# jby1993/SelfReconCode

Measured on AMD Instinct MI355X. Metric: train.py-equivalent iterations/sec (540x540, 2048 rays/frame x 3 frames per GPU; coarse stage at Adam lr 0.0001), higher is better.
Workload: dtype f32

## Files before the change

include/selfrecon_hip.h:

```cpp
#ifndef SELFRECON_HIP_H_
#define SELFRECON_HIP_H_
#include <stdint.h>

#ifdef __cplusplus
extern "C" {
#endif

#define SR_OK 0
#define SR_EINVAL (-1)
#define SR_ELAUNCH (-2)
#define SR_ENOSPC (-3)

int sr_abi_version(void);
const char* sr_build_arch(void);
const char* sr_build_digest(void);

int sr_minv3x3_fwd_f32(const float* ms, float* invs, uint8_t* checks, int64_t n, void* stream);
int sr_minv3x3_fwd_f64(const double* ms, double* invs, uint8_t* checks, int64_t n, void* stream);
int sr_minv3x3_bwd_f32(const float* grads, const float* invs, float* outs, int64_t n, void* stream);
int sr_minv3x3_bwd_f64(const double* grads, const double* invs, double* outs, int64_t n, void* stream);

typedef struct {
  int64_t size[5];
  int64_t stride[5];
// ... 19 lines not shown
                             void* grad_grad_output, void* stream);
int sr_gridsample3d_dbwd_f32(const float* gO_input , sr_tensor5 goi_d, const float* gO_grid, sr_tensor5 gog_d,
                             const float* input, sr_tensor5 in_d, const float* grid, sr_tensor5 grid_d,
                             const float* grad_output, sr_tensor5 gout_d,
                             float* grad_input , sr_tensor5 gin_d, float* grad_grid, float* grad_grad_output,
                             void* stream);
int sr_gridsample3d_dbwd_f64(const double* gO_input , sr_tensor5 goi_d, const double* gO_grid, sr_tensor5 gog_d,
                             const double* input, sr_tensor5 in_d, const double* grid, sr_tensor5 grid_d,
                             const double* grad_output, sr_tensor5 gout_d,
                             double* grad_input , sr_tensor5 gin_d, double* grad_grid, double* grad_grad_output,
                             void* stream);


#define SR_ACT_NONE 0
#define SR_ACT_SOFTPLUS100 1
#define SR_ACT_RELU 2
#define SR_EPI_FWD 0
#define SR_EPI_BWD 1
typedef struct {
  const float* A; int64_t lda;
  const float* B; int64_t ldb;
  float* C; int64_t ldc;
  int32_t M, N, K;
  const float* bias;
  int32_t group, act, mode;
  float out_scale;
  const float* aux; int64_t ldaux;
  int32_t naux_fwd;
  int32_t nact_bwd;
  float aux_scale;
} sr_gemm_args;
int sr_mlp_gemm_nt(const sr_gemm_args* host_args, void* stream);
int sr_mlp_gemm_nt_tile(int32_t M, int32_t ncols, int32_t* bm_out, int32_t* bn_out);

#define SR_CHAIN_MAX_LAYERS 10
typedef struct {
  int32_t nlayers;
  int32_t nprob[SR_CHAIN_MAX_LAYERS];
  sr_gemm_args g[SR_CHAIN_MAX_LAYERS][2];
  const int32_t* m_dev; int32_t m_mul;
  int32_t m_cap;
} sr_chain_args;
int sr_mlp_chain(const sr_chain_args* host_args, void* stream);

typedef struct {
  const float* Z; int64_t ldz;
  const float* A; int64_t lda;
  float* dW; int64_t lddw;
  float* partial;
  int32_t R, N, K, splits, accumulate;
  float* db; float* db_partial; int32_t group;
} sr_gemm_tn_args;
int64_t sr_mlp_gemm_tn_workspace_floats(int32_t R, int32_t N, int64_t lddw, int32_t* host_splits_out);
int sr_mlp_gemm_tn(const sr_gemm_tn_args* host_args, void* stream);
#define SR_TN_GROUP_MAX 12
typedef struct {
  int32_t n;
  sr_gemm_tn_args p[SR_TN_GROUP_MAX];
} sr_gemm_tn_group_args;
int sr_mlp_gemm_tn_group(const sr_gemm_tn_group_args* host_args, void* stream);

int sr_pe_embed(const float* x, int64_t P, int32_t L, const float* band_weights, const float* extra, int64_t ldextra,
                int32_t E, const int64_t* extra_index , int32_t group, float* out, int64_t ldo, void* stream);
int sr_pe_embed_bwd(const float* x, int64_t P, int32_t L, const float* band_weights, int32_t group, const float* gA0,
                    int64_t ldg, float* xbar, void* stream);

typedef struct {
  const float* p; const float* tp; int64_t P;
  const float* A; const float* trans; int32_t nframes;
  const int64_t* batch_inds; int64_t points_per_frame;
  const float* vol; int32_t D, H, W;
  float bmin[3], bmax[3];
  float* y;
  float* jac;
} sr_lbs_args;
int sr_lbs_fwd(const sr_lbs_args* host_args, void* stream);
int64_t sr_lbs_bwd_workspace_floats(int64_t P, int32_t nframes);
int sr_lbs_bwd(const sr_lbs_args* host_args, const float* ybar, float* pbar, float* Abar, float* transbar, float* partials, void* stream);
int sr_lbs_jac_bwd(const sr_lbs_args* host_args, const float* ybar, const float* Jbar, float* pbar, float* Abar, float* transbar, float* partials,
                   void* stream);

int sr_lbs_chain_fwd(const float* poses, int32_t B, const float* host_Js, const int32_t* host_parents, const float* host_init_pose,
                     float* G, float* A, void* stream);
int sr_lbs_chain_bwd(const float* poses, int32_t B, const float* host_Js, const int32_t* host_parents, const float* host_init_pose,
                     const float* Abar, const float* Gbar, float* posebar, void* stream);

typedef struct {
// ... 183 lines not shown
```

selfreconcode_amd/_lib.py:

```python
import ctypes
import os
import torch

from .build import LIB

_i64, _vp, _int = ctypes.c_int64, ctypes.c_void_p, ctypes.c_int


class SrTensor5(ctypes.Structure):
    _fields_ = [("size", _i64 * 5), ("stride", _i64 * 5)]


class SrGemmArgs(ctypes.Structure):
    _fields_ = [("A", _vp), ("lda", _i64), ("B", _vp), ("ldb", _i64), ("C", _vp), ("ldc", _i64),
                ("M", ctypes.c_int32), ("N", ctypes.c_int32), ("K", ctypes.c_int32), ("bias", _vp),
                ("group", ctypes.c_int32), ("act", ctypes.c_int32), ("mode", ctypes.c_int32), ("out_scale", ctypes.c_float),
                ("aux", _vp), ("ldaux", _i64), ("naux_fwd", ctypes.c_int32), ("nact_bwd", ctypes.c_int32),
                ("aux_scale", ctypes.c_float)]


class SrGemmTnArgs(ctypes.Structure):
    _fields_ = [("Z", _vp), ("ldz", _i64), ("A", _vp), ("lda", _i64), ("dW", _vp), ("lddw", _i64), ("partial", _vp),
                ("R", ctypes.c_int32), ("N", ctypes.c_int32), ("K", ctypes.c_int32), ("splits", ctypes.c_int32),
                ("accumulate", ctypes.c_int32), ("db", _vp), ("db_partial", _vp), ("group", ctypes.c_int32)]
# ... 98 lines not shown
_CODES = {-1: "SR_EINVAL (bad argument)", -2: "SR_ELAUNCH (kernel launch failed)", -3: "SR_ENOSPC (workspace too small)"}

if "SELFRECON_HIP_LIB" in os.environ:
    LIB = os.environ["SELFRECON_HIP_LIB"]
else:
    from .build import is_stale, build_lib
    if is_stale():
        try:
            build_lib(verbose=False)
        except RuntimeError as e:
            raise ImportError(str(e)) from e
if not os.path.isfile(LIB):
    raise ImportError(f"{LIB} not found: run `python -m selfreconcode_amd.build` (hipcc --offload-arch=gfx950). "
                      "There is no CPU fallback for the HIP hot path.")
_lib = ctypes.CDLL(LIB)

_T5 = SrTensor5
SIGNATURES = {
    "sr_minv3x3_fwd_f32": [_vp, _vp, _vp, _i64, _vp],
    "sr_minv3x3_fwd_f64": [_vp, _vp, _vp, _i64, _vp],
    "sr_minv3x3_bwd_f32": [_vp, _vp, _vp, _i64, _vp],
    "sr_minv3x3_bwd_f64": [_vp, _vp, _vp, _i64, _vp],
    "sr_gridsample3d_fwd_f16": [_vp, _T5, _vp, _T5, _vp, _T5, _vp],
    "sr_gridsample3d_bwd_f16": [_vp, _T5, _vp, _T5, _vp, _T5, _vp, _T5, _vp, _vp],
    "sr_gridsample3d_dbwd_f16": [_vp, _T5, _vp, _T5, _vp, _T5, _vp, _T5, _vp, _T5, _vp, _T5, _vp, _vp, _vp],
    "sr_gridsample3d_fwd_f32": [_vp, _T5, _vp, _T5, _vp, _T5, _vp],
    "sr_gridsample3d_fwd_f64": [_vp, _T5, _vp, _T5, _vp, _T5, _vp],
    "sr_gridsample3d_bwd_f32": [_vp, _T5, _vp, _T5, _vp, _T5, _vp, _T5, _vp, _vp],
    "sr_gridsample3d_bwd_f64": [_vp, _T5, _vp, _T5, _vp, _T5, _vp, _T5, _vp, _vp],
    "sr_gridsample3d_dbwd_f32": [_vp, _T5, _vp, _T5, _vp, _T5, _vp, _T5, _vp, _T5, _vp, _T5, _vp, _vp, _vp],
    "sr_gridsample3d_dbwd_f64": [_vp, _T5, _vp, _T5, _vp, _T5, _vp, _T5, _vp, _T5, _vp, _T5, _vp, _vp, _vp],
    "sr_mlp_gemm_nt": [_vp, _vp],
    "sr_mlp_gemm_nt_tile": [ctypes.c_int32, ctypes.c_int32, _vp, _vp],
    "sr_mlp_chain": [_vp, _vp],
    "sr_refine_init": [_vp, _vp],
    "sr_refine_embed": [_vp, ctypes.c_int32, _vp],
    "sr_refine_mid": [_vp, ctypes.c_int32, ctypes.c_int32, _vp],
    "sr_refine_finish": [_vp, ctypes.c_int32, _vp],
    "sr_mlp_gemm_tn_workspace_floats": [ctypes.c_int32, ctypes.c_int32, _i64, _vp],
    "sr_mlp_gemm_tn": [_vp, _vp],
    "sr_mlp_gemm_tn_group": [_vp, _vp],
    "sr_lbs_chain_fwd": [_vp, ctypes.c_int32, _vp, _vp, _vp, _vp, _vp, _vp],
    "sr_lbs_chain_bwd": [_vp, ctypes.c_int32, _vp, _vp, _vp, _vp, _vp, _vp, _vp],
    "sr_lbs_fwd": [_vp, _vp],
    "sr_lbs_bwd_workspace_floats": [_i64, ctypes.c_int32],
    "sr_lbs_bwd": [_vp, _vp, _vp, _vp, _vp, _vp, _vp],
    "sr_lbs_jac_bwd": [_vp, _vp, _vp, _vp, _vp, _vp, _vp, _vp],
    "sr_newton_update": [_vp, _vp],
    "sr_newton_prepare": [_vp, _vp],
    "sr_newton_apply": [_vp, _vp],
    "sr_mc_workspace_bytes": [ctypes.c_int32, ctypes.c_int32, ctypes.c_int32],
    "sr_mc_count": [_vp, ctypes.c_int32, ctypes.c_int32, ctypes.c_int32, ctypes.c_float, _vp, _vp, _vp],
    "sr_mc_emit": [_vp, ctypes.c_int32, ctypes.c_int32, ctypes.c_int32, ctypes.c_float, _vp] + [ctypes.c_float] * 6 + [_vp, _vp, _vp],
    "sr_rows_pad": [_vp, _i64, ctypes.c_int32, _vp, _i64, ctypes.c_int32, _i64, ctypes.c_int32, _vp, _i64, ctypes.c_int32, _vp],
    "sr_rows_frame_sum_workspace_floats": [_i64, ctypes.c_int32, ctypes.c_int32],
    "sr_rows_frame_sum": [_vp, _i64, _i64, ctypes.c_int32, _vp, ctypes.c_int32, _vp, _vp, _vp],
    "sr_adam_step": [_vp, _vp],
    "sr_stream_stamp": [_vp, _vp],
    "sr_stream_flag_set": [_vp, ctypes.c_uint32, _vp],
    "sr_stream_flag_wait": [_vp, ctypes.c_uint32, _vp, ctypes.c_int32, _vp],
    "sr_pack_weights": [_vp, _vp],
    "sr_unpack_grads": [_vp, _vp],
    "sr_svd3x3": [_vp, _i64, _vp, _vp, _vp, _vp],
    "sr_step_reduce_blocks": [_i64],
    "sr_step_param_blocks": [_i64],
    "sr_cam_project_ndc_fwd": [_vp, _i64, _vp, _vp, _vp, _vp],
    "sr_cam_project_ndc_bwd": [_vp, _i64, _vp, _vp, _vp, _vp, _vp, _vp, _vp],
    "sr_cam_view_rays_fwd": [_vp, _i64, _vp, _vp, _vp],
    "sr_cam_view_rays_bwd": [_vp, _i64, _vp, _vp, _vp, _vp, _vp],
    "sr_cardinal_rays_fwd": [_vp, _vp, _i64, _vp, _vp, _vp],
    "sr_cardinal_rays_bwd": [_vp, _vp, _i64, _vp, _vp, _vp, _vp],
    "sr_deformed_normals": [_vp, _vp, _i64, _vp, _vp],
    "sr_color_loss_fwd": [_vp, _vp, _vp, _vp, _vp, _vp],
# ... 172 lines not shown
```

selfreconcode_amd/csrc/mlp_gemm.hip:

```cpp
#include "sr_common.h"
#include <stdlib.h>
#include <type_traits>

typedef float f32x16 __attribute__((ext_vector_type(16)));
typedef float f32x4 __attribute__((ext_vector_type(4)));
typedef int i32x4 __attribute__((ext_vector_type(4)));

__device__ __forceinline__ __amdgpu_buffer_rsrc_t sr_make_rsrc(const void* base, int64_t bytes) {
  return __builtin_amdgcn_make_buffer_rsrc(const_cast<void*>(base), 0, (int)(bytes < 0xFFFFFFFFll ? bytes : 0xFFFFFFFFll), 0x00020000);
}
__device__ __forceinline__ f32x4 sr_buffer_load16(__amdgpu_buffer_rsrc_t rsrc, uint32_t lane_off, uint32_t scalar_off) {
  return __builtin_bit_cast(f32x4, __builtin_amdgcn_raw_buffer_load_b128(rsrc, (int)lane_off, (int)scalar_off, 0));
}

namespace {

constexpr int BK = 32;
constexpr int LDSP = BK + 4;

__device__ __forceinline__ float fast_exp(float x) { return __builtin_amdgcn_exp2f(x * 1.4426950408889634f); }
__device__ __forceinline__ float fast_log(float x) { return __builtin_amdgcn_logf(x) * 0.6931471805599453f; }
__device__ __forceinline__ float softplus100(float z) {
  const float t = z * 100.0f;
  const float e = fast_exp(fminf(t, 20.0f));
  const float l = e < 1e-3f ? e * (1.0f - e * (0.5f - e * 0.33333334f)) : fast_log(1.0f + e);
  return t > 20.0f ? z : l * 0.01f;
}
__device__ __forceinline__ float dsoftplus100(float z) {
  const float t = z * 100.0f;
  const float e = fast_exp(fminf(t, 20.0f));
  return t > 20.0f ? 1.0f : e * __builtin_amdgcn_rcpf(e + 1.0f);
}
__device__ __forceinline__ void softplus100_from_stored(float x, float& d, float& c2) {
  const float em = fast_exp(-x);
// ... 190 lines not shown
            if constexpr (ACT == SR_ACT_SOFTPLUS100) softplus100_from_stored(100.0f * (sv[s] * inv_as), d, c2);
            else if constexpr (ACT == SR_ACT_RELU) d = sv[s] > 0.f ? 1.f : 0.f;
            float cross = 0.f;
#pragma unroll
            for (int tI = 1; tI < G; ++tI) {
              cross += sv[s + tI] * v[s + tI];
              o[s + tI] = d * as * v[s + tI];
            }
            o[s] = d * as * v[s] + c2 * cross;
          }
        }
        float* sp = stage + (a * 32 + 8 * q + 4 * kh) * SP + b * 32 + li;
#pragma unroll
        for (int j = 0; j < 4; ++j) sp[j * SP] = o[j];
      }
    }
  }
  __syncthreads();
  constexpr int QPR = TN * 8, RPI = 64 / QPR;
  const int lane = kh * 32 + li;
  const int qc = lane % QPR, ro = lane / QPR;
  float* dst = g.C + (int64_t)(m0 + wm * TM * 32 + ro) * g.ldc + n0 + wn * TN * 32 + qc * 4;
#pragma unroll
  for (int i = 0; i < TM * 32 / RPI; ++i)
    *reinterpret_cast<f32x4*>(dst + (int64_t)i * RPI * g.ldc) = *reinterpret_cast<const f32x4*>(stage + (i * RPI + ro) * SP + qc * 4);
}

template <int WM, int WN, int TM, int TN, int G, int MODE>
__device__ __forceinline__ void epilogue_interior_act(const sr_gemm_args& g, f32x16 (&acc)[TM][TN], int m0, int n0, int wm, int wn, int li,
                                                      int kh, float* __restrict__ stage) {
  if (g.act == SR_ACT_SOFTPLUS100) epilogue_interior<WM, WN, TM, TN, G, MODE, SR_ACT_SOFTPLUS100>(g, acc, m0, n0, wm, wn, li, kh, stage);
  else if (g.act == SR_ACT_RELU) epilogue_interior<WM, WN, TM, TN, G, MODE, SR_ACT_RELU>(g, acc, m0, n0, wm, wn, li, kh, stage);
  else epilogue_interior<WM, WN, TM, TN, G, MODE, SR_ACT_NONE>(g, acc, m0, n0, wm, wn, li, kh, stage);
}

struct NoProbe { __device__ __forceinline__ void operator()(int) const {} };
template <int WM, int WN, int TM, int TN, bool KTAIL = true, class Probe = NoProbe>
__device__ __forceinline__ void gemm_nt_tile(const sr_gemm_args& g, int wg, float* __restrict__ smem, Probe probe = Probe()) {
  using C_ = Cfg<WM, WN, TM, TN>;
  auto As = [&](int buf) -> float* { return smem + buf * (C_::BM * LDSP); };
  auto Bs = [&](int buf) -> float* { return smem + 2 * C_::BM * LDSP + buf * (C_::BN * LDSP); };

  const int tiles_n = (g.N + g.naux_fwd + C_::BN - 1) / C_::BN;
  const int tiles_m = (g.M + C_::BM - 1) / C_::BM;
  const int nwg = tiles_m * tiles_n;
  {
    const int q = nwg / 8, r = nwg % 8, xcd = wg % 8, loc = wg / 8;
    wg = (xcd < r ? xcd * (q + 1) : r * (q + 1) + (xcd - r) * q) + loc;
  }
  const int tn = wg % tiles_n, tm = wg / tiles_n;
  const int m0 = tm * C_::BM, n0 = tn * C_::BN;

  const int lane = threadIdx.x & 63, wave = threadIdx.x >> 6;
  const int wm = wave / WN, wn = wave % WN;
  const int li = lane & 31, kh = lane >> 5;

  f32x16 acc[TM][TN];
#pragma unroll
  for (int a = 0; a < TM; ++a)
#pragma unroll
    for (int b = 0; b < TN; ++b)
#pragma unroll
      for (int r = 0; r < 16; ++r) acc[a][b][r] = 0.f;

  const TileLoader<C_::BM, C_::kALoads, C_::kThreads> la(g.A, g.lda, g.M, g.K, m0);
  const TileLoader<C_::BN, C_::kBLoads, C_::kThreads> lb(g.B, g.ldb, g.N, g.K, n0);
// ... 40 lines not shown
    mfma_kk(fa0[0], fb0[0]);
    mfma_kk(fa0[1], fb0[1]);
#pragma unroll
    for (int i = 0; i < kMem; ++i) {
      __builtin_amdgcn_sched_group_barrier(0x020, 1, 0);
      __builtin_amdgcn_sched_group_barrier(0x008, 1, 0);
    }
#pragma unroll
    for (int i = 0; i < kMem; ++i) {
      __builtin_amdgcn_sched_group_barrier(0x200, 1, 0);
      __builtin_amdgcn_sched_group_barrier(0x008, 1, 0);
    }
#pragma unroll
    for (int i = 0; i < 2 * (TM + TN); ++i) {
      __builtin_amdgcn_sched_group_barrier(0x100, 1, 0);
      __builtin_amdgcn_sched_group_barrier(0x008, 1, 0);
    }
    __builtin_amdgcn_sched_barrier(0);
    __syncthreads();
    read_frags(As(cur ^ 1), Bs(cur ^ 1), 0, fa0, fb0);
    __builtin_amdgcn_sched_barrier(0);
    mfma_kk(fa1[0], fb1[0]);
    mfma_kk(fa1[1], fb1[1]);
    __builtin_amdgcn_sched_barrier(0);
  };
  for (int t = 0; t < nk; t += 2) {
    step(t, ra0, rb0, ra1, rb1);
    if (t + 1 < nk) step(t + 1, ra1, rb1, ra0, rb0);
  }
  __syncthreads();
  probe(1);

  float* stage = smem + wave * (TM * 32 * (TN * 32 + 4));
  const bool interior = m0 + C_::BM <= g.M && n0 + C_::BN <= (g.mode == SR_EPI_FWD ? g.N : (g.nact_bwd < g.N ? g.nact_bwd : g.N));
  if (interior) {
    if (g.mode == SR_EPI_FWD) {
      switch (g.group) {
        case 1: epilogue_interior_act<WM, WN, TM, TN, 1, SR_EPI_FWD>(g, acc, m0, n0, wm, wn, li, kh, stage); break;
        case 2: epilogue_interior_act<WM, WN, TM, TN, 2, SR_EPI_FWD>(g, acc, m0, n0, wm, wn, li, kh, stage); break;
        default: epilogue_interior_act<WM, WN, TM, TN, 4, SR_EPI_FWD>(g, acc, m0, n0, wm, wn, li, kh, stage); break;
      }
    } else {
      switch (g.group) {
        case 1: epilogue_interior_act<WM, WN, TM, TN, 1, SR_EPI_BWD>(g, acc, m0, n0, wm, wn, li, kh, stage); break;
        case 2: epilogue_interior_act<WM, WN, TM, TN, 2, SR_EPI_BWD>(g, acc, m0, n0, wm, wn, li, kh, stage); break;
        default: epilogue_interior_act<WM, WN, TM, TN, 4, SR_EPI_BWD>(g, acc, m0, n0, wm, wn, li, kh, stage); break;
      }
    }
  } else {
    switch (g.group) {
      case 1: epilogue<WM, WN, TM, TN, 1>(g, acc, m0, n0, wm, wn, li, kh, stage); break;
      case 2: epilogue<WM, WN, TM, TN, 2>(g, acc, m0, n0, wm, wn, li, kh, stage); break;
      default: epilogue<WM, WN, TM, TN, 4>(g, acc, m0, n0, wm, wn, li, kh, stage); break;
    }
  }
  probe(2);
}

template <int WM, int WN, int TM, int TN, bool KTAIL>
__global__ __launch_bounds__(WM * WN * 64) __attribute__((amdgpu_waves_per_eu(2))) void gemm_nt_kernel(sr_gemm_args g) {
  extern __shared__ __attribute__((aligned(16))) float smem[];
  gemm_nt_tile<WM, WN, TM, TN, KTAIL>(g, blockIdx.x, smem);
}


using ChainCfg = Cfg<2, 2, 1, 1>;

constexpr int TBR = 32;
template <int ZW, int XW>
struct TnCfg {
  static constexpr int ZLD = ZW + 4, XLD = XW + 4;
  static constexpr int kZ = TBR * ZLD, kX = TBR * XLD;
  static constexpr int kLdsFloats = 2 * (kZ + kX);
  static constexpr int TLZ = TBR * (ZW / 4) / 256, TLX = TBR * (XW / 4) / 256;
  static constexpr int WN = XW / 64;
};

template <int ZW, int XW>
__device__ __forceinline__ void gemm_tn_body(const sr_gemm_tn_args& g, int rows_per_split, int bid, int nblocks, float* __restrict__ tn_smem) {
  using C = TnCfg<ZW, XW>;
  auto Zs = [&](int buf) -> float* { return tn_smem + buf * C::kZ; };
  auto Xs = [&](int buf) -> float* { return tn_smem + 2 * C::kZ + buf * C::kX; };
  const int tiles_k = (g.K + XW - 1) / XW;
  const int tiles_n = (g.N + ZW - 1) / ZW;
  int vb = bid;
  if ((nblocks & 7) == 0) vb = (bid & 7) * (nblocks >> 3) + (bid >> 3);
  const int tile = vb % (tiles_k * tiles_n), split = vb / (tiles_k * tiles_n);
  const int n0 = (tile / tiles_k) * ZW, k0 = (tile % tiles_k) * XW;
  const int r_begin = split * rows_per_split;
  const int r_end = min(g.R, r_begin + rows_per_split);
  const int lane = threadIdx.x & 63, wave = threadIdx.x >> 6;
  const int wm = wave / C::WN, wn = wave % C::WN, li = lane & 31, kh = lane >> 5;

  f32x16 acc[2][2];
#pragma unroll
  for (int a = 0; a < 2; ++a)
#pragma unroll
// ... 241 lines not shown
}

__global__ __launch_bounds__(256) void slab_reduce_group_kernel(TnGroup G) {
  int i = 0;
  while (i + 1 < G.n && (int)blockIdx.x >= G.first[i + 1]) ++i;
  const int bid = blockIdx.x - G.first[i];
  if (bid >= G.blocks[i]) return;
  const sr_gemm_tn_args& g = G.p[i];
  slab_reduce_body(g.partial, g.dW, g.N, g.K, g.lddw, g.R > 0 ? g.splits : 0, g.accumulate, g.db_partial, g.db, bid, G.blocks[i]);
}

}

static void nt_tile_choice(int M, int ncols, int* bm, int* bn) {
  auto cost = [&](int tm, int tn, double eff) {
    const int64_t wgs = sr_cdiv(M, tm) * sr_cdiv(ncols, tn);
    return (double)sr_cdiv(wgs, 256) * tm * tn / eff;
  };
  if (ncols <= 32) {
    const double c[3] = {cost(32, 32, 0.6), cost(64, 32, 0.8), cost(256, 32, 1.0)};
    *bn = 32;
    if (c[0] < c[1] && c[0] < c[2]) *bm = 32;
    else if (c[1] < c[2]) *bm = 64;
    else *bm = 256;
  } else {
    const double c[3] = {cost(64, 64, 0.92), cost(64, 128, 0.94), cost(128, 128, 1.0)};
    int pick = 1;
    for (int i = 1; i < 3; ++i) if (c[i] < c[pick - 1]) pick = i + 1;
    *bm = pick == 3 ? 128 : 64;
    *bn = pick == 1 ? 64 : 128;
  }
}

extern "C" {
int sr_mlp_gemm_nt(const sr_gemm_args* a, void* stream) {
  if (!a || a->M < 0 || a->N <= 0 || a->K <= 0) return SR_EINVAL;
  if (a->M == 0) return SR_OK;
  if (!a->A || !a->B || !a->C) return SR_EINVAL;
  if (a->group != 1 && a->group != 2 && a->group != 4) return SR_EINVAL;
  if ((a->lda & 3) || (a->ldb & 3) || (a->ldc & 3) || ((uintptr_t)a->A & 15) || ((uintptr_t)a->B & 15) || ((uintptr_t)a->C & 15)) return SR_EINVAL;
  if (a->mode != SR_EPI_FWD && a->mode != SR_EPI_BWD) return SR_EINVAL;
  if ((a->naux_fwd > 0 || a->mode == SR_EPI_BWD) && a->act != SR_ACT_NONE && !a->aux && a->mode == SR_EPI_BWD) return SR_EINVAL;
  if (a->mode == SR_EPI_FWD && a->naux_fwd > 0 && !a->aux) return SR_EINVAL;
  if (a->M == 0) return SR_OK;
  if (a->M % a->group) return SR_EINVAL;
  const int ncols = a->N + (a->mode == SR_EPI_FWD ? a->naux_fwd : 0);
  sr_gemm_args g = *a;
  if (g.mode != SR_EPI_FWD) g.naux_fwd = 0;
#define SR_NT_LAUNCH(WM, WN, TM, TN)                                                                                        \
  do {                                                                                                                      \
    using C_ = Cfg<WM, WN, TM, TN>;                                                                                         \
    const int nwg = (int)(sr_cdiv(g.M, C_::BM) * sr_cdiv(ncols, C_::BN));                                                   \
    if (g.K % BK)                                                                                                           \
      hipLaunchKernelGGL((gemm_nt_kernel<WM, WN, TM, TN, true>), dim3(nwg), dim3(C_::kThreads), C_::kLdsFloats * sizeof(float), \
                         (hipStream_t)stream, g);                                                                           \
    else                                                                                                                    \
      hipLaunchKernelGGL((gemm_nt_kernel<WM, WN, TM, TN, false>), dim3(nwg), dim3(C_::kThreads), C_::kLdsFloats * sizeof(float), \
                         (hipStream_t)stream, g);                                                                           \
  } while (0)
  int bm = 0, bn = 0;
  nt_tile_choice(g.M, ncols, &bm, &bn);
  switch (bm * 1024 + bn) {
    case 32 * 1024 + 32: SR_NT_LAUNCH(1, 1, 1, 1); break;
    case 64 * 1024 + 32: SR_NT_LAUNCH(2, 1, 1, 1); break;
    case 256 * 1024 + 32: SR_NT_LAUNCH(4, 1, 2, 1); break;
    case 64 * 1024 + 64: SR_NT_LAUNCH(2, 2, 1, 1); break;
    case 64 * 1024 + 128: SR_NT_LAUNCH(2, 2, 1, 2); break;
    default: SR_NT_LAUNCH(2, 2, 2, 2); break;
  }
#undef SR_NT_LAUNCH
  return sr_launch_status();
}

int sr_mlp_gemm_nt_tile(int32_t M, int32_t ncols, int32_t* bm, int32_t* bn) {
  if (M <= 0 || ncols <= 0 || !bm || !bn) return SR_EINVAL;
  nt_tile_choice(M, ncols, bm, bn);
  return SR_OK;
}

__global__ __launch_bounds__(ChainCfg::kThreads) __attribute__((amdgpu_waves_per_eu(2))) void mlp_layer_pair_kernel(sr_gemm_args g0, sr_gemm_args g1, int nprob,
                                                                                                                     const int32_t* __restrict__ m_dev, int m_mul) {
  extern __shared__ __attribute__((aligned(16))) float smem[];
  const int M = *m_dev * m_mul;
  if (M <= 0) return;
  const int rows = (M + ChainCfg::BM - 1) / ChainCfg::BM;
  const int t0 = rows * ((g0.N + (g0.mode == SR_EPI_FWD ? g0.naux_fwd : 0) + ChainCfg::BN - 1) / ChainCfg::BN);
  const int t1 = nprob > 1 ? rows * ((g1.N + (g1.mode == SR_EPI_FWD ? g1.naux_fwd : 0) + ChainCfg::BN - 1) / ChainCfg::BN) : 0;
  const int t = blockIdx.x;
  if (t >= t0 + t1) return;
  if (t < t0) { g0.M = M; if (g0.K % BK) gemm_nt_tile<2, 2, 1, 1, true>(g0, t, smem); else gemm_nt_tile<2, 2, 1, 1, false>(g0, t, smem); }
  else { g1.M = M; if (g1.K % BK) gemm_nt_tile<2, 2, 1, 1, true>(g1, t - t0, smem); else gemm_nt_tile<2, 2, 1, 1, false>(g1, t - t0, smem); }
}

int sr_mlp_chain(const sr_chain_args* a, void* stream) {
  if (!a || a->nlayers < 1 || a->nlayers > SR_CHAIN_MAX_LAYERS || !a->m_dev || a->m_mul < 1 || a->m_cap <= 0) return SR_EINVAL;
  for (int l = 0; l < a->nlayers; ++l) {
    if (a->nprob[l] < 1 || a->nprob[l] > 2) return SR_EINVAL;
    for (int p = 0; p < a->nprob[l]; ++p) {
      const sr_gemm_args& g = a->g[l][p];
      if (!g.A || !g.B || !g.C || g.N <= 0 || g.K <= 0 || g.group != a->m_mul) return SR_EINVAL;
      if ((g.lda & 3) || (g.ldb & 3) || (g.ldc & 3) || ((uintptr_t)g.A & 15) || ((uintptr_t)g.B & 15) || ((uintptr_t)g.C & 15)) return SR_EINVAL;
      if (g.mode != SR_EPI_FWD && g.mode != SR_EPI_BWD) return SR_EINVAL;
      if (g.mode == SR_EPI_BWD && g.naux_fwd != 0) return SR_EINVAL;
      if ((g.mode == SR_EPI_BWD && g.act != SR_ACT_NONE && !g.aux) || (g.mode == SR_EPI_FWD && g.naux_fwd > 0 && !g.aux)) return SR_EINVAL;
    }
  }
  const int64_t rows = sr_cdiv((int64_t)a->m_cap * a->m_mul, ChainCfg::BM);
  for (int l = 0; l < a->nlayers; ++l) {
    int64_t tiles = 0;
    for (int p = 0; p < a->nprob[l]; ++p) {
      const sr_gemm_args& g = a->g[l][p];
      tiles += rows * sr_cdiv(g.N + (g.mode == SR_EPI_FWD ? g.naux_fwd : 0), ChainCfg::BN);
    }
    hipLaunchKernelGGL(mlp_layer_pair_kernel, dim3((unsigned)tiles), dim3(ChainCfg::kThreads), ChainCfg::kLdsFloats * sizeof(float), (hipStream_t)stream,
                       a->g[l][0], a->g[l][a->nprob[l] > 1 ? 1 : 0], a->nprob[l], a->m_dev, a->m_mul);
  }
  return sr_launch_status();
}

int64_t sr_mlp_gemm_tn_workspace_floats(int32_t R, int32_t N, int64_t lddw, int32_t* splits_out) {
  const int tiles = tn_narrow(N, lddw) ? (int)sr_cdiv(N, 256) : (int)(sr_cdiv(N, 128) * sr_cdiv(lddw, 128));
  const int target = 512;
  int splits = (int)sr_cdiv(target, tiles);
  const int max_splits = (int)sr_cdiv(R, 384);
  if (splits > max_splits) splits = max_splits;
  if (splits < 1) splits = 1;
  if (splits_out) *splits_out = splits;
  return (int64_t)splits * N * lddw;
}

int sr_mlp_gemm_tn(const sr_gemm_tn_args* a, void* stream) {
  if (!a || !a->dW || !a->partial || a->R < 0 || a->N <= 0 || a->K <= 0 || a->splits < 1) return SR_EINVAL;
  if (a->R > 0 && (!a->Z || !a->A)) return SR_EINVAL;
  if ((a->ldz & 3) || (a->lda & 3) || ((uintptr_t)a->Z & 15) || ((uintptr_t)a->A & 15) || a->lddw < a->K) return SR_EINVAL;
  if ((a->lddw & 3) || ((uintptr_t)a->dW & 15) || ((uintptr_t)a->partial & 15)) return SR_EINVAL;
  if ((a->db != nullptr) != (a->db_partial != nullptr) || (a->db && a->group < 1)) return SR_EINVAL;
  const bool narrow = tn_narrow(a->N, a->lddw);
  const int tiles = narrow ? (int)sr_cdiv(a->N, 256) : (int)(sr_cdiv(a->N, 128) * sr_cdiv(a->K, 128));
  int rows_per_split = (int)sr_cdiv(a->R, a->splits);
  rows_per_split = (int)(sr_cdiv(rows_per_split, TBR) * TBR);
  if (a->R > 0) {
    using Narrow = TnCfg<256, 64>;
    using Square = TnCfg<128, 128>;
    if (narrow)
      hipLaunchKernelGGL((gemm_tn_kernel<256, 64>), dim3(tiles * a->splits), dim3(256), Narrow::kLdsFloats * sizeof(float), (hipStream_t)stream, *a,
                         rows_per_split);
    else
      hipLaunchKernelGGL((gemm_tn_kernel<128, 128>), dim3(tiles * a->splits), dim3(256), Square::kLdsFloats * sizeof(float), (hipStream_t)stream, *a,
                         rows_per_split);
  }
  const int64_t total = (int64_t)a->N * a->lddw / 4 + (a->db ? a->N : 0);
  hipLaunchKernelGGL(slab_reduce_kernel, dim3(sr_stream_grid(total, 256)), dim3(256), 0, (hipStream_t)stream, a->partial, a->dW,
                     a->N, a->K, a->lddw, a->R > 0 ? a->splits : 0, a->accumulate, a->db_partial, a->db);
  return sr_launch_status();
}

static int tn_check(const sr_gemm_tn_args* a) {
  if (!a || !a->dW || !a->partial || a->R < 0 || a->N <= 0 || a->K <= 0 || a->splits < 1) return SR_EINVAL;
  if (a->R > 0 && (!a->Z || !a->A)) return SR_EINVAL;
  if ((a->ldz & 3) || (a->lda & 3) || ((uintptr_t)a->Z & 15) || ((uintptr_t)a->A & 15) || a->lddw < a->K) return SR_EINVAL;
  if ((a->lddw & 3) || ((uintptr_t)a->dW & 15) || ((uintptr_t)a->partial & 15)) return SR_EINVAL;
  if ((a->db != nullptr) != (a->db_partial != nullptr) || (a->db && a->group < 1)) return SR_EINVAL;
  return SR_OK;
}

int sr_mlp_gemm_tn_group(const sr_gemm_tn_group_args* a, void* stream) {
  if (!a || a->n < 1 || a->n > SR_TN_GROUP_MAX) return SR_EINVAL;
  TnGroup G, Rd;
  G.n = Rd.n = a->n;
  int nb = 0, nr = 0;
  bool any_rows = false;
  for (int i = 0; i < a->n; ++i) {
    const sr_gemm_tn_args& p = a->p[i];
    const int rc = tn_check(&p);
    if (rc != SR_OK) return rc;
    if (tn_narrow(p.N, p.lddw)) return SR_EINVAL;
    const int tiles = (int)(sr_cdiv(p.N, 128) * sr_cdiv(p.K, 128));
    int rows_per_split = (int)sr_cdiv(p.R, p.splits);
    rows_per_split = (int)(sr_cdiv(rows_per_split, TBR) * TBR);
    G.p[i] = Rd.p[i] = p;
    G.rows_per_split[i] = Rd.rows_per_split[i] = rows_per_split;
    G.first[i] = nb; G.blocks[i] = p.R > 0 ? tiles * p.splits : 0;
    nb += (int)(sr_cdiv(G.blocks[i], 8) * 8);
    const int64_t total = (int64_t)p.N * p.lddw / 4 + (p.db ? p.N : 0);
    Rd.first[i] = nr; Rd.blocks[i] = sr_stream_grid(total, 256);
    nr += Rd.blocks[i];
    any_rows = any_rows || p.R > 0;
  }
  G.first[a->n] = nb; Rd.first[a->n] = nr;
  using Square = TnCfg<128, 128>;
  if (any_rows && nb > 0)
    hipLaunchKernelGGL(gemm_tn_group_kernel, dim3(nb), dim3(256), Square::kLdsFloats * sizeof(float), (hipStream_t)stream, G);
  hipLaunchKernelGGL(slab_reduce_group_kernel, dim3(nr), dim3(256), 0, (hipStream_t)stream, Rd);
  return sr_launch_status();
}
}

// ... 79 lines not shown
```

selfreconcode_amd/mlp_engine.py:

```python
import collections
import contextlib
import ctypes
import math
import os
import weakref
import torch

from . import _lib

ACT_NONE, ACT_SOFTPLUS100, ACT_RELU = 0, 1, 2
EPI_FWD, EPI_BWD = 0, 1

TN_SIDE_STREAM = True
GROUP_TN_BELOW = 16384
DEBUG_TN_DELAY_MS = int(os.environ.get("SR_DEBUG_TN_DELAY_MS", "0"))
_TN_STREAMS = {}
_TN_PENDING = set()
_DELAY_FLAG = {}

DEFERRED_PARAM_GRADS = False

_PACK_CACHE = {}
_ENTRY_BY_PTR = {}

# ... 138 lines not shown
    set_gemm_args(a, A, B, C, M, N, K, bias, group, act, mode, out_scale, aux, naux_fwd, nact_bwd, aux_scale, (lda, ldb, ldc, ldaux))
    PROFILE.launch("sr_mlp_gemm_nt", a, _lib.stream_of(C), M >= 128 and N > 32, (M, N, K, mode, group))


_TnProblem = collections.namedtuple("_TnProblem", "Z ldz A lda R N K lddw group dW db accumulate")


def _tn_workspace(R, N, lddw):
    splits = ctypes.c_int32(0)
    ws = _lib.raw("sr_mlp_gemm_tn_workspace_floats")(R, N, lddw, ctypes.byref(splits))
    return max(int(ws), 1), splits.value


def _set_tn_args(a, Z, ldz, A, lda, R, N, K, lddw, group, dW, db, accumulate, partial, ws, splits):
    a.Z, a.ldz, a.A, a.lda, a.dW, a.lddw, a.partial = Z.data_ptr(), ldz, A.data_ptr(), lda, dW.data_ptr(), lddw, partial
    a.R, a.N, a.K, a.splits, a.accumulate = R, N, K, splits, 1 if accumulate else 0
    a.db, a.db_partial, a.group = db.data_ptr(), partial + 4 * ws, group


def _gemm_tn(Z, ldz, A, lda, R, N, K, lddw, group=1, dW=None, db=None, accumulate=False):
    ws, splits = _tn_workspace(R, N, lddw)
    if dW is None:
        dW = torch.empty((N, lddw), dtype=torch.float32, device=Z.device)
    partial = torch.empty((ws + splits * N,), dtype=torch.float32, device=Z.device)
    if db is None:
        db = torch.empty((N,), dtype=torch.float32, device=Z.device)
    a = _lib.SrGemmTnArgs()
    _set_tn_args(a, Z, ldz, A, lda, R, N, K, lddw, group, dW, db, accumulate, partial.data_ptr(), ws, splits)
    PROFILE.launch("sr_mlp_gemm_tn", a, _lib.stream_of(Z), R >= 128 and N > 32, (R, N, K, "tn", group))
    return dW, db


def _tn_is_narrow(N, lddw):
    return lddw <= 64 and N >= 256


def _gemm_tn_group(problems):
    problems = [_TnProblem(*p) for p in problems]
    g = _lib.SrGemmTnGroupArgs()
    g.n = len(problems)
    sizes, total = [], 0
    for p in problems:
        ws, splits = _tn_workspace(p.R, p.N, p.lddw)
        sizes.append((ws, splits, total))
        total += (ws + splits * p.N + 3) // 4 * 4
    partial = torch.empty((total,), dtype=torch.float32, device=problems[0].Z.device)
    for a, p, (ws, splits, off) in zip(g.p, problems, sizes):
        _set_tn_args(a, *p, partial.data_ptr() + 4 * off, ws, splits)
    _lib.call("sr_mlp_gemm_tn_group", ctypes.byref(g), _lib.stream_of(partial))


def _debug_delay(device, ms):
    f = _DELAY_FLAG.get(str(device))
    if f is None:
        f = _DELAY_FLAG[str(device)] = torch.zeros(2, dtype=torch.int32, device=device)
    _lib.call('sr_stream_flag_wait', f.data_ptr(), 0x40000000, 0, ms, torch.cuda.current_stream(device).cuda_stream)


def _tn_stream(device):
    key = str(device)
    st = _TN_STREAMS.get(key)
    if st is None:
        st = _TN_STREAMS[key] = torch.cuda.Stream(device=device)
    return st


def _launch_on_tn_stream(device, problems):
# ... 540 lines not shown
```

Before: 23.48.

## Add register-resident streaming NT GEMM kernel for small-K forward layers

Adds a persistent streaming GEMM kernel for forward-mode NT problems with N>=256 and K<=40. Each block keeps its B (weight) fragments in registers and loops over 32-row panels of A, prefetching the next panel while running the epilogue. The goal is to avoid repeated LDS staging and per-tile weight reloads for wide, shallow layers such as the positional-embedding input layer. The change also tightens argument validation (leading dimensions, 32-bit extents) and moves the narrow-TN predicate into C. The stream kernel now replaces the tiled path for every matching shape, since the minimum row count is 1, so small-M cases may be slower.

```diff
diff --git a/include/selfrecon_hip.h b/include/selfrecon_hip.h
--- a/include/selfrecon_hip.h
+++ b/include/selfrecon_hip.h
@@ -75,6 +75,9 @@
 } sr_gemm_args;
 int sr_mlp_gemm_nt(const sr_gemm_args* host_args, void* stream);
 int sr_mlp_gemm_nt_tile(int32_t M, int32_t ncols, int32_t* bm_out, int32_t* bn_out);
+int sr_mlp_gemm_nt_general(const sr_gemm_args* host_args, void* stream);
+int sr_mlp_gemm_nt_stream(const sr_gemm_args* host_args, void* stream);
+int sr_mlp_gemm_nt_stream_min_rows(int32_t N, int32_t K, int32_t mode);
 
 #define SR_CHAIN_MAX_LAYERS 10
 typedef struct {
@@ -96,6 +99,7 @@
 } sr_gemm_tn_args;
 int64_t sr_mlp_gemm_tn_workspace_floats(int32_t R, int32_t N, int64_t lddw, int32_t* host_splits_out);
 int sr_mlp_gemm_tn(const sr_gemm_tn_args* host_args, void* stream);
+int sr_mlp_tn_is_narrow(int32_t N, int64_t lddw);
 #define SR_TN_GROUP_MAX 12
 typedef struct {
   int32_t n;
diff --git a/selfreconcode_amd/_lib.py b/selfreconcode_amd/_lib.py
--- a/selfreconcode_amd/_lib.py
+++ b/selfreconcode_amd/_lib.py
@@ -154,6 +154,9 @@
     "sr_gridsample3d_dbwd_f64": [_vp, _T5, _vp, _T5, _vp, _T5, _vp, _T5, _vp, _T5, _vp, _T5, _vp, _vp, _vp],
     "sr_mlp_gemm_nt": [_vp, _vp],
     "sr_mlp_gemm_nt_tile": [ctypes.c_int32, ctypes.c_int32, _vp, _vp],
+    "sr_mlp_gemm_nt_general": [_vp, _vp],
+    "sr_mlp_gemm_nt_stream": [_vp, _vp],
+    "sr_mlp_gemm_nt_stream_min_rows": [ctypes.c_int32, ctypes.c_int32, ctypes.c_int32],
     "sr_mlp_chain": [_vp, _vp],
     "sr_refine_init": [_vp, _vp],
     "sr_refine_embed": [_vp, ctypes.c_int32, _vp],
@@ -161,6 +164,7 @@
     "sr_refine_finish": [_vp, ctypes.c_int32, _vp],
     "sr_mlp_gemm_tn_workspace_floats": [ctypes.c_int32, ctypes.c_int32, _i64, _vp],
     "sr_mlp_gemm_tn": [_vp, _vp],
+    "sr_mlp_tn_is_narrow": [ctypes.c_int32, _i64],
     "sr_mlp_gemm_tn_group": [_vp, _vp],
     "sr_lbs_chain_fwd": [_vp, ctypes.c_int32, _vp, _vp, _vp, _vp, _vp, _vp],
     "sr_lbs_chain_bwd": [_vp, ctypes.c_int32, _vp, _vp, _vp, _vp, _vp, _vp, _vp],
diff --git a/selfreconcode_amd/csrc/mlp_gemm.hip b/selfreconcode_amd/csrc/mlp_gemm.hip
--- a/selfreconcode_amd/csrc/mlp_gemm.hip
+++ b/selfreconcode_amd/csrc/mlp_gemm.hip
@@ -1,5 +1,6 @@
 #include "sr_common.h"
 #include <stdlib.h>
+#include <algorithm>
 #include <type_traits>
 
 typedef float f32x16 __attribute__((ext_vector_type(16)));
@@ -256,6 +257,34 @@
   if (g.act == SR_ACT_SOFTPLUS100) epilogue_interior<WM, WN, TM, TN, G, MODE, SR_ACT_SOFTPLUS100>(g, acc, m0, n0, wm, wn, li, kh, stage);
   else if (g.act == SR_ACT_RELU) epilogue_interior<WM, WN, TM, TN, G, MODE, SR_ACT_RELU>(g, acc, m0, n0, wm, wn, li, kh, stage);
   else epilogue_interior<WM, WN, TM, TN, G, MODE, SR_ACT_NONE>(g, acc, m0, n0, wm, wn, li, kh, stage);
+}
+
+template <int WM, int WN, int TM, int TN>
+__device__ __forceinline__ void nt_epilogue(const sr_gemm_args& g, f32x16 (&acc)[TM][TN], int m0, int n0, int wm, int wn, int li, int kh,
+                                            float* __restrict__ stage) {
+  using C_ = Cfg<WM, WN, TM, TN>;
+  const bool interior = m0 + C_::BM <= g.M && n0 + C_::BN <= (g.mode == SR_EPI_FWD ? g.N : (g.nact_bwd < g.N ? g.nact_bwd : g.N));
+  if (interior) {
+    if (g.mode == SR_EPI_FWD) {
+      switch (g.group) {
+        case 1: epilogue_interior_act<WM, WN, TM, TN, 1, SR_EPI_FWD>(g, acc, m0, n0, wm, wn, li, kh, stage); break;
+        case 2: epilogue_interior_act<WM, WN, TM, TN, 2, SR_EPI_FWD>(g, acc, m0, n0, wm, wn, li, kh, stage); break;
+        default: epilogue_interior_act<WM, WN, TM, TN, 4, SR_EPI_FWD>(g, acc, m0, n0, wm, wn, li, kh, stage); break;
+      }
+    } else {
+      switch (g.group) {
+        case 1: epilogue_interior_act<WM, WN, TM, TN, 1, SR_EPI_BWD>(g, acc, m0, n0, wm, wn, li, kh, stage); break;
+        case 2: epilogue_interior_act<WM, WN, TM, TN, 2, SR_EPI_BWD>(g, acc, m0, n0, wm, wn, li, kh, stage); break;
+        default: epilogue_interior_act<WM, WN, TM, TN, 4, SR_EPI_BWD>(g, acc, m0, n0, wm, wn, li, kh, stage); break;
+      }
+    }
+  } else {
+    switch (g.group) {
+      case 1: epilogue<WM, WN, TM, TN, 1>(g, acc, m0, n0, wm, wn, li, kh, stage); break;
+      case 2: epilogue<WM, WN, TM, TN, 2>(g, acc, m0, n0, wm, wn, li, kh, stage); break;
+      default: epilogue<WM, WN, TM, TN, 4>(g, acc, m0, n0, wm, wn, li, kh, stage); break;
+    }
+  }
 }
 
 struct NoProbe { __device__ __forceinline__ void operator()(int) const {} };
@@ -362,28 +391,7 @@
   probe(1);
 
   float* stage = smem + wave * (TM * 32 * (TN * 32 + 4));
-  const bool interior = m0 + C_::BM <= g.M && n0 + C_::BN <= (g.mode == SR_EPI_FWD ? g.N : (g.nact_bwd < g.N ? g.nact_bwd : g.N));
-  if (interior) {
-    if (g.mode == SR_EPI_FWD) {
-      switch (g.group) {
-        case 1: epilogue_interior_act<WM, WN, TM, TN, 1, SR_EPI_FWD>(g, acc, m0, n0, wm, wn, li, kh, stage); break;
-        case 2: epilogue_interior_act<WM, WN, TM, TN, 2, SR_EPI_FWD>(g, acc, m0, n0, wm, wn, li, kh, stage); break;
-        default: epilogue_interior_act<WM, WN, TM, TN, 4, SR_EPI_FWD>(g, acc, m0, n0, wm, wn, li, kh, stage); break;
-      }
-    } else {
-      switch (g.group) {
-        case 1: epilogue_interior_act<WM, WN, TM, TN, 1, SR_EPI_BWD>(g, acc, m0, n0, wm, wn, li, kh, stage); break;
-        case 2: epilogue_interior_act<WM, WN, TM, TN, 2, SR_EPI_BWD>(g, acc, m0, n0, wm, wn, li, kh, stage); break;
-        default: epilogue_interior_act<WM, WN, TM, TN, 4, SR_EPI_BWD>(g, acc, m0, n0, wm, wn, li, kh, stage); break;
-      }
-    }
-  } else {
-    switch (g.group) {
-      case 1: epilogue<WM, WN, TM, TN, 1>(g, acc, m0, n0, wm, wn, li, kh, stage); break;
-      case 2: epilogue<WM, WN, TM, TN, 2>(g, acc, m0, n0, wm, wn, li, kh, stage); break;
-      default: epilogue<WM, WN, TM, TN, 4>(g, acc, m0, n0, wm, wn, li, kh, stage); break;
-    }
-  }
+  nt_epilogue<WM, WN, TM, TN>(g, acc, m0, n0, wm, wn, li, kh, stage);
   probe(2);
 }
 
@@ -393,6 +401,72 @@
   gemm_nt_tile<WM, WN, TM, TN, KTAIL>(g, blockIdx.x, smem);
 }
 
+
+template <int NKK>
+struct StreamCfg {
+  static constexpr int WM = 1, WN = 4, TM = 1, TN = 4;
+  using C_ = Cfg<WM, WN, TM, TN>;
+  static constexpr int kLdsFloats = C_::kStageFloats;
+  static constexpr int kMaxK = NKK * 8;
+  static constexpr int kResident = 512;
+};
+
+__device__ __forceinline__ f32x4 stream_frag_load(const float* __restrict__ p, int k, int kmax) {
+  return *reinterpret_cast<const f32x4*>(p + (k < kmax ? k : kmax));
+}
+__device__ __forceinline__ f32x4 stream_frag_mask(f32x4 v, int nvalid) {
+  v.x = nvalid > 0 ? v.x : 0.f; v.y = nvalid > 1 ? v.y : 0.f; v.z = nvalid > 2 ? v.z : 0.f; v.w = nvalid > 3 ? v.w : 0.f;
+  return v;
+}
+
+template <int NKK>
+__global__ __launch_bounds__(256) __attribute__((amdgpu_waves_per_eu(2))) void gemm_nt_stream_kernel(sr_gemm_args g, int tiles_n, int panels) {
+  using S = StreamCfg<NKK>;
+  extern __shared__ __attribute__((aligned(16))) float smem[];
+  const int lane = threadIdx.x & 63, wave = threadIdx.x >> 6;
+  const int li = lane & 31, kh = lane >> 5;
+  const int n0 = ((int)blockIdx.x % tiles_n) * S::C_::BN;
+  const int stride = (int)gridDim.x / tiles_n;
+  const int kmax = ((g.K + 3) & ~3) - 4;
+  float* stage = smem + wave * (S::TM * 32 * (S::TN * 32 + 4));
+
+  f32x4 fb[S::TN][NKK];
+#pragma unroll
+  for (int b = 0; b < S::TN; ++b) {
+    int row = n0 + (wave * S::TN + b) * 32 + li;
+    row = row < g.N ? row : g.N - 1;
+    const float* bp = g.B + (int64_t)row * g.ldb;
+#pragma unroll
+    for (int kk = 0; kk < NKK; ++kk) fb[b][kk] = stream_frag_mask(stream_frag_load(bp, kk * 8 + kh * 4, kmax), g.K - (kk * 8 + kh * 4));
+  }
+  auto load_a = [&](int panel, f32x4 (&fa)[NKK]) {
+    int row = panel * 32 + li;
+    row = row < g.M ? row : g.M - 1;
+    const float* ap = g.A + (int64_t)row * g.lda;
+#pragma unroll
+    for (int kk = 0; kk < NKK; ++kk) fa[kk] = stream_frag_load(ap, kk * 8 + kh * 4, kmax);
+  };
+  int panel = (int)blockIdx.x / tiles_n;
+  f32x4 fa[NKK];
+  if (panel < panels) load_a(panel, fa);
+  for (; panel < panels; panel += stride) {
+    f32x16 acc[S::TM][S::TN];
+#pragma unroll
+    for (int b = 0; b < S::TN; ++b)
+#pragma unroll
+      for (int r = 0; r < 16; ++r) acc[0][b][r] = 0.f;
+#pragma unroll
+    for (int kk = 0; kk < NKK; ++kk) {
+      const f32x4 a4 = stream_frag_mask(fa[kk], g.K - (kk * 8 + kh * 4));
+#pragma unroll
+      for (int e = 0; e < 4; ++e)
+#pragma unroll
+        for (int b = 0; b < S::TN; ++b) acc[0][b] = __builtin_amdgcn_mfma_f32_32x32x2f32(a4[e], fb[b][kk][e], acc[0][b], 0, 0, 0);
+    }
+    if (panel + stride < panels) load_a(panel + stride, fa);
+    nt_epilogue<S::WM, S::WN, S::TM, S::TN>(g, acc, panel * 32, n0, 0, wave, li, kh, stage);
+  }
+}
 
 using ChainCfg = Cfg<2, 2, 1, 1>;
 
@@ -700,21 +774,24 @@
   }
 }
 
-extern "C" {
-int sr_mlp_gemm_nt(const sr_gemm_args* a, void* stream) {
-  if (!a || a->M < 0 || a->N <= 0 || a->K <= 0) return SR_EINVAL;
-  if (a->M == 0) return SR_OK;
+static inline bool sr_extent_ok(int64_t rows, int64_t ld) { return rows * ld * 4 < (int64_t(1) << 32); }
+
+static int nt_check(const sr_gemm_args* a, bool rows_from_device) {
+  if (!a || a->N <= 0 || a->K <= 0 || (!rows_from_device && a->M < 0)) return SR_EINVAL;
+  if (!rows_from_device && a->M == 0) return SR_OK;
   if (!a->A || !a->B || !a->C) return SR_EINVAL;
   if (a->group != 1 && a->group != 2 && a->group != 4) return SR_EINVAL;
   if ((a->lda & 3) || (a->ldb & 3) || (a->ldc & 3) || ((uintptr_t)a->A & 15) || ((uintptr_t)a->B & 15) || ((uintptr_t)a->C & 15)) return SR_EINVAL;
   if (a->mode != SR_EPI_FWD && a->mode != SR_EPI_BWD) return SR_EINVAL;
-  if ((a->naux_fwd > 0 || a->mode == SR_EPI_BWD) && a->act != SR_ACT_NONE && !a->aux && a->mode == SR_EPI_BWD) return SR_EINVAL;
+  if (a->mode == SR_EPI_BWD && a->act != SR_ACT_NONE && !a->aux) return SR_EINVAL;
   if (a->mode == SR_EPI_FWD && a->naux_fwd > 0 && !a->aux) return SR_EINVAL;
-  if (a->M == 0) return SR_OK;
-  if (a->M % a->group) return SR_EINVAL;
-  const int ncols = a->N + (a->mode == SR_EPI_FWD ? a->naux_fwd : 0);
-  sr_gemm_args g = *a;
-  if (g.mode != SR_EPI_FWD) g.naux_fwd = 0;
+  if (a->naux_fwd < 0 || a->lda < a->K || a->ldb < a->K || a->ldc < (int64_t)a->N + (a->mode == SR_EPI_FWD ? a->naux_fwd : 0)) return SR_EINVAL;
+  if (!sr_extent_ok(256, a->lda) || !sr_extent_ok(256, a->ldb)) return SR_EINVAL;
+  if (!rows_from_device && a->M % a->group) return SR_EINVAL;
+  return SR_OK;
+}
+
+static void nt_launch_tiles(const sr_gemm_args& g, int ncols, void* stream) {
 #define SR_NT_LAUNCH(WM, WN, TM, TN)                                                                                        \
   do {                                                                                                                      \
     using C_ = Cfg<WM, WN, TM, TN>;                                                                                         \
@@ -737,7 +814,39 @@
     default: SR_NT_LAUNCH(2, 2, 2, 2); break;
   }
 #undef SR_NT_LAUNCH
+}
+
+static bool nt_stream_shape(const sr_gemm_args& g) { return g.mode == SR_EPI_FWD && g.N >= 256 && g.K <= StreamCfg<5>::kMaxK; }
+static constexpr int kStreamMinRows = 1;
+
+static void nt_launch_stream(const sr_gemm_args& g, int ncols, void* stream) {
+  using S = StreamCfg<5>;
+  const int tiles_n = (int)sr_cdiv(ncols, S::C_::BN), panels = (int)sr_cdiv(g.M, S::C_::BM);
+  const int per_col = std::max(1, std::min(panels, S::kResident / tiles_n));
+  hipLaunchKernelGGL((gemm_nt_stream_kernel<5>), dim3(per_col * tiles_n), dim3(256), S::kLdsFloats * sizeof(float), (hipStream_t)stream, g, tiles_n, panels);
+}
+
+static int nt_entry(const sr_gemm_args* a, void* stream, int which) {
+  const int rc = nt_check(a, false);
+  if (rc != SR_OK || a->M == 0) return rc;
+  const int ncols = a->N + (a->mode == SR_EPI_FWD ? a->naux_fwd : 0);
+  sr_gemm_args g = *a;
+  if (g.mode != SR_EPI_FWD) g.naux_fwd = 0;
+  const bool shape = which != 1 && nt_stream_shape(g);
+  if (which == 2 && !shape) return SR_EINVAL;
+  if (shape && (which == 2 || g.M >= kStreamMinRows)) nt_launch_stream(g, ncols, stream);
+  else nt_launch_tiles(g, ncols, stream);
   return sr_launch_status();
+}
+
+extern "C" {
+int sr_mlp_gemm_nt(const sr_gemm_args* a, void* stream) { return nt_entry(a, stream, 0); }
+int sr_mlp_gemm_nt_general(const sr_gemm_args* a, void* stream) { return nt_entry(a, stream, 1); }
+int sr_mlp_gemm_nt_stream(const sr_gemm_args* a, void* stream) { return nt_entry(a, stream, 2); }
+int sr_mlp_gemm_nt_stream_min_rows(int32_t N, int32_t K, int32_t mode) {
+  sr_gemm_args g = {};
+  g.N = N; g.K = K; g.mode = mode;
+  return nt_stream_shape(g) ? kStreamMinRows : -1;
 }
 
 int sr_mlp_gemm_nt_tile(int32_t M, int32_t ncols, int32_t* bm, int32_t* bn) {
@@ -771,6 +880,8 @@
       if (g.mode != SR_EPI_FWD && g.mode != SR_EPI_BWD) return SR_EINVAL;
       if (g.mode == SR_EPI_BWD && g.naux_fwd != 0) return SR_EINVAL;
       if ((g.mode == SR_EPI_BWD && g.act != SR_ACT_NONE && !g.aux) || (g.mode == SR_EPI_FWD && g.naux_fwd > 0 && !g.aux)) return SR_EINVAL;
+      if (g.naux_fwd < 0 || g.lda < g.K || g.ldb < g.K || g.ldc < (int64_t)g.N + (g.mode == SR_EPI_FWD ? g.naux_fwd : 0)) return SR_EINVAL;
+      if (!sr_extent_ok(ChainCfg::BM, g.lda) || !sr_extent_ok(ChainCfg::BN, g.ldb)) return SR_EINVAL;
     }
   }
   const int64_t rows = sr_cdiv((int64_t)a->m_cap * a->m_mul, ChainCfg::BM);
@@ -797,12 +908,22 @@
   return (int64_t)splits * N * lddw;
 }
 
-int sr_mlp_gemm_tn(const sr_gemm_tn_args* a, void* stream) {
+static int tn_check(const sr_gemm_tn_args* a) {
   if (!a || !a->dW || !a->partial || a->R < 0 || a->N <= 0 || a->K <= 0 || a->splits < 1) return SR_EINVAL;
   if (a->R > 0 && (!a->Z || !a->A)) return SR_EINVAL;
   if ((a->ldz & 3) || (a->lda & 3) || ((uintptr_t)a->Z & 15) || ((uintptr_t)a->A & 15) || a->lddw < a->K) return SR_EINVAL;
   if ((a->lddw & 3) || ((uintptr_t)a->dW & 15) || ((uintptr_t)a->partial & 15)) return SR_EINVAL;
   if ((a->db != nullptr) != (a->db_partial != nullptr) || (a->db && a->group < 1)) return SR_EINVAL;
+  if (a->R > 0) {
+    const int64_t rows_per_split = sr_cdiv(sr_cdiv(a->R, a->splits), TBR) * TBR;
+    if (a->ldz < a->N || a->lda < a->K || !sr_extent_ok(rows_per_split, a->ldz) || !sr_extent_ok(rows_per_split, a->lda)) return SR_EINVAL;
+  }
+  return SR_OK;
+}
+
+int sr_mlp_gemm_tn(const sr_gemm_tn_args* a, void* stream) {
+  const int rc = tn_check(a);
+  if (rc != SR_OK) return rc;
   const bool narrow = tn_narrow(a->N, a->lddw);
   const int tiles = narrow ? (int)sr_cdiv(a->N, 256) : (int)(sr_cdiv(a->N, 128) * sr_cdiv(a->K, 128));
   int rows_per_split = (int)sr_cdiv(a->R, a->splits);
@@ -823,14 +944,7 @@
   return sr_launch_status();
 }
 
-static int tn_check(const sr_gemm_tn_args* a) {
-  if (!a || !a->dW || !a->partial || a->R < 0 || a->N <= 0 || a->K <= 0 || a->splits < 1) return SR_EINVAL;
-  if (a->R > 0 && (!a->Z || !a->A)) return SR_EINVAL;
-  if ((a->ldz & 3) || (a->lda & 3) || ((uintptr_t)a->Z & 15) || ((uintptr_t)a->A & 15) || a->lddw < a->K) return SR_EINVAL;
-  if ((a->lddw & 3) || ((uintptr_t)a->dW & 15) || ((uintptr_t)a->partial & 15)) return SR_EINVAL;
-  if ((a->db != nullptr) != (a->db_partial != nullptr) || (a->db && a->group < 1)) return SR_EINVAL;
-  return SR_OK;
-}
+int sr_mlp_tn_is_narrow(int32_t N, int64_t lddw) { return tn_narrow(N, lddw) ? 1 : 0; }
 
 int sr_mlp_gemm_tn_group(const sr_gemm_tn_group_args* a, void* stream) {
   if (!a || a->n < 1 || a->n > SR_TN_GROUP_MAX) return SR_EINVAL;
diff --git a/selfreconcode_amd/mlp_engine.py b/selfreconcode_amd/mlp_engine.py
--- a/selfreconcode_amd/mlp_engine.py
+++ b/selfreconcode_amd/mlp_engine.py
@@ -194,7 +194,7 @@
 
 
 def _tn_is_narrow(N, lddw):
-    return lddw <= 64 and N >= 256
+    return bool(_lib.raw("sr_mlp_tn_is_narrow")(N, lddw))
 
 
 def _gemm_tn_group(problems):
```

Measured after the change: 23.37, median of 2. Within noise of the previous version (-0.4%).
